# UofgCoastline/EUSIPCO-2026-Robust-Unet

Hardware: AMD Instinct MI355X
Metric: train images/sec Robust U-Net 256x256 bs16/GPU (higher is better)
Workload: dtype f32; 1 GPU; Robust U-Net base64 (40.9M params) train step, 256x256 RGB+mask tiles, batch 16/GPU, fp32, BCE + Adam(lr 1e-4, wd 1e-4), dropout + batch-stat BN on; global_batch=16, image_size=256, parallelism=dp1

## Files before the change

### eusipco-2026-robust-unet_amd/ops.py

```python
from __future__ import annotations

import ctypes
import os
import threading
import weakref

import torch

from ._lib import check, lib

CONV_FWD, CONV_DGRAD, CONVT_FWD, CONVT_DGRAD, CONV_DGRAD_T, CONVT_DGRAD_T = 0, 1, 2, 3, 4, 5

_ws = {}
PIN_SCRATCH = False
_retired = []


def grow(pool, key, nfloats, device, floor):
    buf = pool.get(key)
    if buf is None or buf.numel() < nfloats:
        if buf is not None and PIN_SCRATCH:
            _retired.append(buf)
        buf = torch.empty(max(int(nfloats), floor, 2 * buf.numel() if buf is not None else 0), device=device, dtype=torch.float32)
        if getattr(_tls, "override", None) is not None:
# ... 298 lines not shown
        return False
    return (USE_WINOGRAD4 and kh == 3 and cin_w == k and max(k, n) >= WINO4_MIN_WIDE and min(k, n) >= WINO4_MIN_NARROW and h * w <= WINO4_MAX_PIXELS
            and bool(lib.runet_wino4_supported(h // dil, w // dil, k, n)))


USE_STEM_KERNELS = os.environ.get("RUNET_NO_STEM_KERNELS", "0") != "1"


def _stem_case(cin, cin_w, cout, kh, dil=1):
    return USE_STEM_KERNELS and cin == 4 and kh in (1, 3) and dil == 1 and bool(lib.runet_stem_supported(cin_w, cout))


def stem_conv(x, w3, w1=None, stats3=None, stats1=None):
    n, h, w, _ = x.shape
    _, _, cin_w, cout = w3.shape
    y3 = empty_nhwc(n, h, w, cout, x)
    y1 = empty_nhwc(n, h, w, cout, x) if w1 is not None else None
    args = (x.data_ptr(), ld(x), w3.data_ptr(), w1.data_ptr() if w1 is not None else None, y3.data_ptr(), ld(y3),
            y1.data_ptr() if y1 is not None else None, ld(y1) if y1 is not None else 0, n, h, w, cin_w, cout)
    if EPILOGUE_STATS and stats3 is not None and (w1 is None or stats1 is not None):
        parts = lib.runet_stem_conv_stats_parts(n, h, w)
        s3 = _stats_buf(stats3, parts, cout, x.device)
        s1 = _stats_buf(stats1, parts, cout, x.device) if w1 is not None else None
        check(lib.runet_stem_conv_stats(*args, s3, s1, stream()))
    else:
        check(lib.runet_stem_conv(*args, stream()))
    return y3, y1


USE_CONV_X3 = os.environ.get("RUNET_NO_CONV_X3", "0") != "1"
CONV_X3_MIN_K = int(os.environ.get("RUNET_CONV_X3_MIN_K", "128"))
CONV_X3_WIDE_N = int(os.environ.get("RUNET_CONV_X3_WIDE_N", "128"))
CONVT_X3_NARROW = os.environ.get("RUNET_NO_CONVT_X3_NARROW", "0") != "1"
_X3_KIND = {CONV_FWD: "cx3f", CONV_DGRAD: "cx3d", CONVT_FWD: "cx3uf", CONVT_DGRAD: "cx3ud"}


def _conv_x3_case(x, cin, cin_w, cout, taps=1):
    k = cin * taps
    return (USE_X3 and USE_CONV_X3 and _PRECISION == "f32" and cin_w == cin and cin % 16 == 0 and cout % 4 == 0 and k >= CONV_X3_MIN_K
            and (k >= 2 * CONV_X3_MIN_K or cout >= CONV_X3_WIDE_N) and ld(x) % 4 == 0 and x.data_ptr() % 16 == 0)


def conv_x3_weights(w_hwio, mode):
    _, _, ci, co = w_hwio.shape
    k, n = (co, ci) if mode in (CONV_DGRAD, CONVT_DGRAD) else (ci, co)
    wp, dev = w_hwio.data_ptr(), w_hwio.device

    def make(out):
        buf = out if out is not None else torch.empty(lib.runet_conv_x3_pack_elems(k, n, mode), device=dev, dtype=torch.bfloat16)
        check(lib.runet_conv_x3_pack(wp, buf.data_ptr(), k, n, mode, stream()))
        return buf
    return _cached(w_hwio, _X3_KIND[mode], make, desc=(DERIVE_PACK, wp, k, n, mode))


EPILOGUE_STATS = os.environ.get("RUNET_NO_EPILOGUE_STATS", "0") != "1"


def _stats_buf(stats, nparts, c, dev):
    part = torch.empty(nparts * c * 3, device=dev, dtype=torch.float32)
    stats["part"], stats["nparts"] = part, nparts
    return part.data_ptr()


def _conv_x3(mode, x, w_hwio, bias, out, n, h, w, cin, cout, accumulate, stats=None):
    wp = conv_x3_weights(w_hwio, mode)
    prof = _PROFILE is not None
    if prof:
        e0, e1 = torch.cuda.Event(enable_timing=True), torch.cuda.Event(enable_timing=True)
        e0.record()
    if stats is not None and EPILOGUE_STATS and mode == CONV_FWD:
        sp = _stats_buf(stats, lib.runet_conv_x3_stats_parts(n, h, w), cout, x.device)
        check(lib.runet_conv_x3_stats(x.data_ptr(), ld(x), wp.data_ptr(), bias.data_ptr() if bias is not None else None, out.data_ptr(), ld(out), n, h, w,
                                      cin, cout, mode, int(accumulate), sp, stream()))
    else:
        check(lib.runet_conv_x3(x.data_ptr(), ld(x), wp.data_ptr(), bias.data_ptr() if bias is not None else None, out.data_ptr(), ld(out), n, h, w,
                                cin, cout, mode, int(accumulate), stream()))
    if prof:
        e1.record()
        fl = 2.0 * n * h * w * (4 if mode in (CONVT_FWD, CONVT_DGRAD) else 1) * cin * cout
        _PROFILE.append((lib.runet_conv_x3_kernel_name(n, h, w, cout, mode).decode(), fl, fl, e0, e1))
    return out


def conv_fwd(x, w_hwio, bias=None, out=None, dil=1, accumulate=False, keep_v=None, stats=None, pre=None):
    n, h, w, cin = x.shape
    kh, kw, cin_w, cout = w_hwio.shape
    if pre is not None:
        assert fuses_act_input(x, w_hwio) and dil == 1
        return wino4_conv(x, wino4_weights(w_hwio), bias, out=out, accumulate=accumulate, keep_v=keep_v, dil=dil, pre=pre, stats=stats)
    if _bf16_case(cin, cin_w):
        if out is None:
            out = empty_nhwc(n, h, w, cout, x)
        return _igemm_bf16(CONV_FWD, x, w_hwio, bias, out, n, h, w, cin, cout, kh, kw, dil, accumulate, False)
    if _wino4_case(h, w, kh, dil, cin, cout, cin_w):
        return wino4_conv(x, wino4_weights(w_hwio), bias, out=out, accumulate=accumulate, keep_v=keep_v, dil=dil, stats=stats)
    if _wino_case(h, w, kh, dil, cin, cout, cin_w, n, ld(x), ld(out) if out is not None else cout):
        return wino_conv(x, wino_weights(w_hwio), bias, out=out, accumulate=accumulate, stats=stats)
    if out is None:
        out = empty_nhwc(n, h, w, cout, x)
    if kh == 1 and _conv_x3_case(x, cin, cin_w, cout):
        return _conv_x3(CONV_FWD, x, w_hwio, bias, out, n, h, w, cin, cout, accumulate, stats=stats)
    _igemm(CONV_FWD, x.data_ptr(), ld(x), w_hwio.data_ptr(), bias.data_ptr() if bias is not None else None,
           out.data_ptr(), ld(out), n, h, w, cin, cin_w, cout, kh, kw, dil, int(accumulate))
    return out


USE_WINO_X3 = os.environ.get("RUNET_NO_WINO_X3", "0") != "1"


def wino_weights(w_hwio, dgrad=False):
    _, _, cin, cout = w_hwio.shape
    k, n = (cout, cin) if dgrad else (cin, cout)
    wp, dev = w_hwio.data_ptr(), w_hwio.device
    if USE_X3 and USE_WINO_X3 and k % 16 == 0:
        def make_x3(out):
            Up = out if out is not None else torch.empty(lib.runet_wino_x3_pack_elems(k, n), device=dev, dtype=torch.bfloat16)
            check(lib.runet_wino_weights_x3(wp, Up.data_ptr(), cin, cout, int(dgrad), stream()))
            Up.kn = (k, n)
            return Up
        return _cached(w_hwio, "wino2xd" if dgrad else "wino2x", make_x3, desc=(DERIVE_WINO2, wp, cin, cout, int(dgrad)))

    def make(out):
        U = out if out is not None else torch.empty((16, k, n), device=dev, dtype=torch.float32)
        check(lib.runet_wino_weights(wp, U.data_ptr(), cin, cout, int(dgrad), stream()))
        return U
    return _cached(w_hwio, "wino2d" if dgrad else "wino2", make)


def wino_conv(x, U, bias=None, out=None, accumulate=False, stats=None):
    n, h, w, k = x.shape
    x3 = U.dtype == torch.bfloat16
    nn_ = U.kn[1] if x3 else U.shape[2]
    if out is None:
        out = empty_nhwc(n, h, w, nn_, x)
    if _PROFILE is not None:
        e0, e1 = torch.cuda.Event(enable_timing=True), torch.cuda.Event(enable_timing=True)
        e0.record()
    if x3 and stats is not None and EPILOGUE_STATS:
        sp = _stats_buf(stats, lib.runet_wino_conv_x3_stats_parts(n, h, w), nn_, x.device)
        check(lib.runet_wino_conv_x3_stats(x.data_ptr(), ld(x), U.data_ptr(), bias.data_ptr() if bias is not None else None, out.data_ptr(), ld(out),
                                           n, h, w, k, nn_, int(accumulate), sp, stream()))
    else:
        fn = lib.runet_wino_conv_x3 if x3 else lib.runet_wino_conv
        check(fn(x.data_ptr(), ld(x), U.data_ptr(), bias.data_ptr() if bias is not None else None, out.data_ptr(), ld(out),
                 n, h, w, k, nn_, int(accumulate), stream()))
    if _PROFILE is not None:
        e1.record()
        fl = 2.0 * n * h * w * 9 * k * nn_
        _PROFILE.append(("wino_conv_x3_kernel" if x3 else "wino_conv_kernel", fl, fl * 16.0 / 36.0, e0, e1))
    return out


def wino_ok(h, w, cin, cout):
    return bool(lib.runet_wino_supported(h, w, cin, cout))


FUSE_BN_INPUT = os.environ.get("RUNET_NO_FUSED_BN_INPUT", "0") != "1"


def fuses_act_input(t, w_hwio):
    n, h, w, cin = t.shape
    kh, kw, cin_w, cout = w_hwio.shape
    return FUSE_BN_INPUT and not _bf16_case(cin, cin_w) and _wino4_case(h, w, kh, 1, cin, cout, cin_w)


def fuses_bn_bwd_input(dy, w_hwio):
    n, h, w, cout = dy.shape
    kh, kw, cin, cout_w = w_hwio.shape
    return (FUSE_BN_INPUT and cout_w == cout and not _bf16_case(cout, cout) and _wino4_case(h, w, kh, 1, cout, cin, cout) and USE_W4_ADJOINT
            and _x3_case(cout) and cin >= 16)


def conv_dgrad(dy, w_hwio, out=None, dil=1, accumulate=False, keep_z=None, bn=None):
    n, h, w, cout = dy.shape
    kh, kw, cin, cout_w = w_hwio.shape
    assert cout_w == cout
    if bn is not None:
        assert fuses_bn_bwd_input(dy, w_hwio) and dil == 1 and keep_z is not None
        return wino4_dgrad_adj(dy, w_hwio, out=out, accumulate=accumulate, dil=dil, keep_z=keep_z, bn=bn)
    if _bf16_case(cout, cout):
        if out is None:
            out = empty_nhwc(n, h, w, cin, dy)
        return _igemm_bf16(CONV_DGRAD, dy, w_hwio, None, out, n, h, w, cout, cin, kh, kw, dil, accumulate, True)
    if _wino4_case(h, w, kh, dil, cout, cin, cout):
        if USE_W4_ADJOINT and _x3_case(cout):
            return wino4_dgrad_adj(dy, w_hwio, out=out, accumulate=accumulate, dil=dil, keep_z=keep_z)
        return wino4_conv(dy, wino4_weights(w_hwio, dgrad=True), None, out=out, accumulate=accumulate, dil=dil)
    if _wino_case(h, w, kh, dil, cout, cin, cout, n, ld(dy), ld(out) if out is not None else cin):
        return wino_conv(dy, wino_weights(w_hwio, dgrad=True), None, out=out, accumulate=accumulate)
    if out is None:
        out = empty_nhwc(n, h, w, cin, dy)
    if kh == 1 and _conv_x3_case(dy, cout, cout, cin):
        return _conv_x3(CONV_DGRAD, dy, w_hwio, None, out, n, h, w, cout, cin, accumulate)
    if USE_TRANSPOSED_DGRAD:
        _igemm(CONV_DGRAD_T, dy.data_ptr(), ld(dy), transposed_weights(w_hwio).data_ptr(), None, out.data_ptr(), ld(out), n, h, w,
               cout, cout, cin, kh, kw, dil, int(accumulate))
    else:
        _igemm(CONV_DGRAD, dy.data_ptr(), ld(dy), w_hwio.data_ptr(), None, out.data_ptr(), ld(out), n, h, w,
               cout, cout, cin, kh, kw, dil, int(accumulate))
    return out


USE_WGRAD_STREAM = os.environ.get("RUNET_NO_WGRAD_STREAM", "0") != "1"
GRAPH_SIDE = os.environ.get("RUNET_GRAPH_SIDE", "0") == "1"
SIDE_RECORD_STREAM = os.environ.get("RUNET_SIDE_RECORD_STREAM", "0") == "1"
_side = {}


class wgrad_side_stream:

    def __enter__(self):
        if USE_WGRAD_STREAM and torch.cuda.is_available() and (GRAPH_SIDE or not torch.cuda.is_current_stream_capturing()):
            dev = torch.cuda.current_device()
            if ("s", dev) not in _side:
                _side[("s", dev)] = torch.cuda.Stream(device=dev)
            _side["active"] = _side[("s", dev)]
            _side["active_raw"] = _side["active"].cuda_stream
            _side["torch_switch"] = torch.cuda.is_current_stream_capturing()
        return self

    def __exit__(self, *exc):
        s = _side.pop("active", None)
        if s is not None:
            torch.cuda.current_stream().wait_stream(s)
        _side.pop("keep", None)
        return False


def side_stream():
    return _side.get("active")


FWD_BRANCHES = os.environ.get("RUNET_FWD_BRANCHES", "1") != "0"
BRANCH_MIN_PIXELS = int(os.environ.get("RUNET_BRANCH_MIN_PIXELS", str(1 << 18)))
_branch_now = True


def branches_pay(n, h, w):
    global _branch_now
    _branch_now = n * h * w >= BRANCH_MIN_PIXELS
    return _branch_now


class side_branch:

    def __init__(self, enabled=True):
        self.s = None
        if (enabled and FWD_BRANCHES and _branch_now and USE_WGRAD_STREAM and torch.cuda.is_available() and _side.get("active") is None
                and not torch.cuda.is_current_stream_capturing()):
            dev = torch.cuda.current_device()
            if ("s", dev) not in _side:
                _side[("s", dev)] = torch.cuda.Stream(device=dev)
            self.s = _side[("s", dev)]

    def __enter__(self):
        if self.s is not None:
            self.s.wait_stream(torch.cuda.current_stream())
            self.ctx = torch.cuda.stream(self.s)
            self.ctx.__enter__()
        return self

    def __exit__(self, *exc):
        if self.s is not None:
            self.ctx.__exit__(*exc)
        return False

    def join(self, *tensors):
        if self.s is not None:
            cur = torch.cuda.current_stream()
            cur.wait_stream(self.s)
            for t in tensors:
                if t is not None and (SIDE_RECORD_STREAM or getattr(t, "_runet_main_pool", False) is False):
                    t.record_stream(cur)
            self.s = None


def main_pool(t):
    t._runet_main_pool = True
    return t


def _on_side(fn, tensors):
    s = _side.get("active")
    if s is None:
        return fn()
    if _PROFILE is not None or _side.get("torch_switch"):
        s.wait_stream(torch.cuda.current_stream())
        with torch.cuda.stream(s):
            r = fn()
    else:
        raw = _side["active_raw"]
        check(lib.runet_stream_wait(raw, stream()))
        _tls.override = raw
        try:
            r = fn()
        finally:
            _tls.override = None
    if SIDE_RECORD_STREAM:
        for t in tensors:
            if t is not None:
                t.record_stream(s)
        return r
    keep = _side.setdefault("keep", [])
    for t in tensors:
        if t is not None:
            keep.append(t)
    return r


def conv_wgrad(x, dy, kh, kw, cin_w=None, dil=1, out=None, v=None, on_side=True, z=None):
    if on_side and _side.get("active") is not None:
        if out is None:
            out = torch.empty((kh, kw, x.shape[3] if cin_w is None else cin_w, dy.shape[3]), device=x.device, dtype=torch.float32)
        return _on_side(lambda: _conv_wgrad(x, dy, kh, kw, cin_w, dil, out, v, z), (x, dy, out, v, z))
    return _conv_wgrad(x, dy, kh, kw, cin_w, dil, out, v, z)


def _conv_wgrad(x, dy, kh, kw, cin_w=None, dil=1, out=None, v=None, z=None):
    n, h, w, cin = x.shape
    cout = dy.shape[3]
    cin_w = cin if cin_w is None else cin_w
    if out is None:
        out = torch.empty((kh, kw, cin_w, cout), device=x.device, dtype=torch.float32)
    if _bf16_case(cin, cin_w):
        return _wgrad_bf16(x, dy, out, n, h, w, cin, cout, kh, kw, dil, 0)
    if _wino4_case(h, w, kh, dil, cin, cout, cin_w) and cout >= 16:
        return wino4_wgrad(x, dy, out=out, v=v, dil=dil, z=z)
    if _stem_case(cin, cin_w, cout, kh, dil):
        ws = workspace(lib.runet_stem_wgrad_workspace_floats(n, h, w, cin_w, cout, kh), x.device)
        check(lib.runet_stem_wgrad(x.data_ptr(), ld(x), dy.data_ptr(), ld(dy), out.data_ptr(), ws.data_ptr(), ws.numel(), n, h, w, cin_w, cout, kh,
                                   stream()))
        return out
    prof = _PROFILE is not None
    if prof:
        e0, e1 = torch.cuda.Event(enable_timing=True), torch.cuda.Event(enable_timing=True)
        e0.record()
    if USE_WINOGRAD and kh == 3 and dil == 1 and cin_w == cin and h % 2 == 0 and w % 2 == 0 and cin >= 16:
        name = "wino_wgrad_direct_kernel(+reduce)"
        nws = lib.runet_wino_wgrad_workspace_floats(n, h, w, cin, cout)
        ws = workspace(nws, x.device)
        check(lib.runet_wino_wgrad(x.data_ptr(), ld(x), dy.data_ptr(), ld(dy), out.data_ptr(), ws.data_ptr(), ws.numel(), n, h, w, cin, cout, stream()))
    else:
        name = "wgrad_tile_kernel/wgrad_kernel(+reduce)"
        nws = lib.runet_conv_wgrad_workspace_floats(n, h, w, cin_w, cout, kh, kw)
        ws = workspace(nws, x.device)
        check(lib.runet_conv_wgrad(x.data_ptr(), ld(x), dy.data_ptr(), ld(dy), out.data_ptr(), ws.data_ptr(), ws.numel(),
                                   n, h, w, cin, cin_w, cout, kh, kw, dil, 0, stream()))
    if prof:
        e1.record()
        fl = 2.0 * n * h * w * kh * kw * cin_w * cout
        _PROFILE.append((name, fl, fl * 16.0 / 36.0 if name.startswith("wino") else fl, e0, e1))
    return out


def _wgrad_bf16(x, dy, out, n, h, w, cin, cout, kh, kw, dil, transposed):
    prof = _PROFILE is not None
    if prof:
        e0, e1 = torch.cuda.Event(enable_timing=True), torch.cuda.Event(enable_timing=True)
        e0.record()
    nws = _lp("runet_conv_wgrad_{}_workspace_floats")(n, h, w, cin, cout, kh, kw, dil, transposed)
    ws = workspace(nws, x.device)
    check(_lp("runet_conv_wgrad_{}")(x.data_ptr(), ld(x), dy.data_ptr(), ld(dy), out.data_ptr(), ws.data_ptr(), ws.numel(), n, h, w, cin, cout,
                                    kh, kw, dil, transposed, stream()))
    if prof:
        e1.record()
        fl = 2.0 * n * h * w * kh * kw * cin * cout
        nbytes = 4.0 * n * h * w * (cin + (4 if transposed else 1) * cout) + 4.0 * kh * kw * cin * cout
        _PROFILE.append((f"wgrad_{_PRECISION}_kernel", fl, fl, e0, e1, nbytes))
    return out


def convt_fwd(x, w_hwio, bias=None, out=None):
    n, h, w, cin = x.shape
    _, _, cin_w, cout = w_hwio.shape
    if out is None:
        out = empty_nhwc(n, 2 * h, 2 * w, cout, x)
    if _bf16_case(cin, cin_w):
        return _igemm_bf16(CONVT_FWD, x, w_hwio, bias, out, n, h, w, cin, cout, 2, 2, 1, False, False)
    if _conv_x3_case(x, cin, cin_w, cout) or (CONVT_X3_NARROW and cout >= 32 and _conv_x3_case(x, cin, cin_w, max(cout, CONV_X3_WIDE_N))):
        return _conv_x3(CONVT_FWD, x, w_hwio, bias, out, n, h, w, cin, cout, False)
    _igemm(CONVT_FWD, x.data_ptr(), ld(x), w_hwio.data_ptr(), bias.data_ptr() if bias is not None else None,
           out.data_ptr(), ld(out), n, h, w, cin, cin_w, cout, 2, 2, 1, 0)
    return out


def convt_dgrad(dy, w_hwio, out=None, accumulate=False):
    n, h2, w2, cout = dy.shape
    _, _, cin, cout_w = w_hwio.shape
    h, w = h2 // 2, w2 // 2
    if out is None:
        out = empty_nhwc(n, h, w, cin, dy)
    if _bf16_case(cout, cout):
        return _igemm_bf16(CONVT_DGRAD, dy, w_hwio, None, out, n, h, w, cout, cin, 2, 2, 1, accumulate, True)
    if _conv_x3_case(dy, cout, cout, cin, taps=4):
        return _conv_x3(CONVT_DGRAD, dy, w_hwio, None, out, n, h, w, cout, cin, accumulate)
    if USE_TRANSPOSED_DGRAD:
        _igemm(CONVT_DGRAD_T, dy.data_ptr(), ld(dy), transposed_weights(w_hwio).data_ptr(), None, out.data_ptr(), ld(out), n, h, w,
               cout, cout, cin, 2, 2, 1, int(accumulate))
    else:
        _igemm(CONVT_DGRAD, dy.data_ptr(), ld(dy), w_hwio.data_ptr(), None, out.data_ptr(), ld(out), n, h, w,
               cout, cout, cin, 2, 2, 1, int(accumulate))
    return out


def convt_wgrad(x, dy, out=None):
    if _side.get("active") is not None:
        if out is None:
            out = torch.empty((2, 2, x.shape[3], dy.shape[3]), device=x.device, dtype=torch.float32)
        return _on_side(lambda: _convt_wgrad(x, dy, out), (x, dy, out))
    return _convt_wgrad(x, dy, out)


def _convt_wgrad(x, dy, out=None):
    n, h, w, cin = x.shape
    cout = dy.shape[3]
    if out is None:
        out = torch.empty((2, 2, cin, cout), device=x.device, dtype=torch.float32)
    if _bf16_case(cin, cin):
        return _wgrad_bf16(x, dy, out, n, h, w, cin, cout, 2, 2, 1, 1)
    nws = lib.runet_conv_wgrad_workspace_floats(n, h, w, cin, cout, 2, 2)
    ws = workspace(nws, x.device)
    check(lib.runet_conv_wgrad(x.data_ptr(), ld(x), dy.data_ptr(), ld(dy), out.data_ptr(), ws.data_ptr(), ws.numel(),
                               n, h, w, cin, cin, cout, 2, 2, 1, 1, stream()))
    return out
# ... 467 lines not shown
```

### include/runet_hip.h

```cpp
#ifndef RUNET_HIP_H
#define RUNET_HIP_H
#ifdef __cplusplus
extern "C" {
#endif

const char* runet_last_error(void);
void runet_set_error(const char* msg);
int runet_abi_version(void);

enum { RUNET_CONV_FWD = 0, RUNET_CONV_DGRAD = 1, RUNET_CONVT_FWD = 2, RUNET_CONVT_DGRAD = 3, RUNET_CONV_DGRAD_T = 4, RUNET_CONVT_DGRAD_T = 5 };

int runet_conv_igemm(const float* x, int ldx, const float* w, const float* bias, float* y, int ldy,
                     int n_img, int h, int w_, int cin, int cin_w, int cout, int kh, int kw, int dil,
                     int mode, int accumulate, void* stream);

int runet_transpose_taps(const float* w, float* wt, int taps, int cin, int cout, void* stream);

const char* runet_conv_igemm_kernel_name(int n_img, int h, int w_, int cin, int cout, int kh, int mode);
int runet_igemm_force_variant(int variant);
int runet_igemm_lowp_force_variant(int variant);

long runet_conv_wgrad_workspace_floats(int n_img, int h, int w_, int cin_w, int cout, int kh, int kw);
int runet_conv_wgrad(const float* x, int ldx, const float* dy, int ldy, float* dw, float* workspace,
                     long workspace_floats, int n_img, int h, int w_, int cin, int cin_w, int cout,
// ... 65 lines not shown
int runet_sa_conv7_bwd(const float* smap, const float* dq, const float* wp, float* dsm, float* dwp, float* workspace, int n_img, int h,
                       int w, void* stream);
int runet_rb_bwd2(const float* dv, int lddv, const float* t2, int ld, const float* sa, const float* dsm, const int* amax, int n_img,
                  int hw, int c, float* workspace, float* sdu, float* sdut, void* stream);
long runet_rb_bwd2_bn_workspace_floats(int n_img, int hw, int c);
int runet_rb_bwd2_bn(const float* dv, int lddv, const float* t2, int ld, const float* sa, const float* dsm, const int* amax, const float* r, int ldr,
                     const float* mean_s, const float* invstd_s, int n_img, int hw, int c, float* workspace, long workspace_floats, float* sdu,
                     float* sdut, float* sums_s, void* stream);
long runet_ca_bwd_workspace_floats(int n_img, int c, int cr);
int runet_ca_bwd(const float* sdu, const float* sdut, const float* s2, const float* h2, const float* ca, const float* avg, const float* mx,
                 const float* w0p, const float* w2p, const float* mean_nc, const float* tval, const float* mean2, const float* invstd2,
                 int n_img, int c, int cr, float* workspace, float* davg, float* dmx, float* sums2, float* dw0p, float* dw2p, void* stream);
int runet_rb_bwd3(const float* dv, int lddv, const float* t2, int ld, const float* sa, const float* dsm, const int* amax, const float* ca,
                  const float* davg, const float* dmx, const int* idx, const float* mean2, const float* invstd2, const float* s2,
                  const float* sums2, float* dt2, int lddt, long pixels, int hw, int c, long m_total, void* stream);
int runet_rb_bwd3_sc(float* dv, int lddv, const float* t2, int ld, const float* sa, const float* dsm, const int* amax, const float* ca,
                     const float* davg, const float* dmx, const int* idx, const float* mean2, const float* invstd2, const float* s2,
                     const float* sums2, float* dt2, int lddt, const float* r, int ldr, const float* mean_s, const float* invstd_s,
                     const float* scale_s, const float* sums_s, long m_total_s, long pixels, int hw, int c, long m_total, void* stream);

int runet_ag_psi(const float* g1, int ldg, const float* x1, int ldx, const float* sg, const float* hg, const float* sx, const float* hx,
                 const float* wpsi, const float* bpsi, float* s, long pixels, int f, void* stream);
int runet_ag_out(const float* xs, int ldx, const float* s, const float* sp, const float* hp, float* out, int ldo, long pixels, int c,
                 void* stream);
int runet_ag_bwd1(const float* datt, int ldd, const float* xs, int ldx, const float* s, const float* sp, const float* hp, float* dxs,
                  int lddx, float* dsbn, long pixels, int c, void* stream);
int runet_ag_bwd2(const float* ds, const float* g1, int ldg, const float* x1, int ldx, const float* sg, const float* hg, const float* sx,
                  const float* hx, const float* wpsi, float* dpre, int ldp, float* workspace, float* dwpsi_db, long pixels, int f,
                  void* stream);
long runet_ag_bwd2_bn_workspace_floats(long pixels, int f);
int runet_ag_bwd2_bn(const float* ds, const float* g1, int ldg, const float* x1, int ldx, const float* sg, const float* hg, const float* sx,
                     const float* hx, const float* wpsi, const float* mean_g, const float* invstd_g, const float* mean_x, const float* invstd_x,
                     float* dpre, int ldp, float* workspace, long workspace_floats, float* dwpsi_db, float* sums_g, float* sums_x, long pixels, int f,
                     void* stream);

int runet_outc_fwd(const float* x, int ld, const float* w, const float* b, float* logit, float* prob, long pixels, int c, void* stream);
int runet_outc_bwd(const float* dprob, const float* prob, const float* x, int ld, const float* w, float* dx, int lddx, float* workspace,
                   float* dw_db, long pixels, int c, void* stream);

int runet_maxpool2_fwd(const float* x, int ldx, float* y, int ldy, unsigned char* idx, int n_img, int h, int w, int c, void* stream);
int runet_maxpool2_bwd(const float* dy, int lddy, const unsigned char* idx, float* dx, int lddx, int n_img, int h, int w, int c,
                       int accumulate, void* stream);
int runet_to_nhwc_pad(const float* x, long sn, long sc, long sh, long sw, float* y, int n_img, int c, int h, int w, int c_pad, void* stream);

int runet_bce_fwd(const float* prob, const float* target, long n, double* workspace1024, float* loss, void* stream);
int runet_bce_bwd(const float* prob, const float* target, const float* grad_out, float* dprob, long n, void* stream);

int runet_adam_chunk_elems(void);
int runet_adam_multi(const long long* table, int n_tensors, const int* chunks, int n_chunks, float lr, float beta1, float beta2, float eps,
                     float weight_decay, int step, float grad_scale, const int* skip_flag, void* stream);

int runet_adam_multi_dev(const long long* table, int n_tensors, const int* chunks, int n_chunks, const float* hyper, int* step_dev,
                         const int* skip_flag, void* stream);
int runet_nonfinite_flag(const float* buf, long n, int* flag2, void* stream);
int runet_stream_wait(void* waiter, void* waited);


int runet_seg_counts(const float* pred, const float* target, long long* counts, int n_img, long per_img, float threshold, void* stream);

int runet_gemm_batched(const float* a, int lda, long stride_a, const float* b, long stride_b, float* c, int ldc, long stride_c, int batch, int rows,
                       int k, int n, void* stream);
int runet_gemm_tn_batched(const float* a, int lda, long stride_a, const float* b, int ldb, long stride_b, float* c, int batch, int rows, int k, int n,
                          int rows_per_split, void* stream);
const char* runet_gemm_batched_kernel_name(int batch, int rows, int k, int n);

int runet_gemm_x3_supported(int rows, int k, int n);
long runet_gemm_x3_pack_elems(int batch, int k, int n);
int runet_gemm_x3_pack(const float* b, long stride_b, void* packed, int batch, int k, int n, void* stream);
int runet_gemm_x3_batched(const float* a, int lda, long stride_a, const void* packed_b, float* c, int ldc, long stride_c, int batch, int rows,
                          int k, int n, void* stream);
int runet_gemm_x3_tn_batched(const float* a, int lda, long stride_a, const float* b, int ldb, long stride_b, float* c, int batch, int rows, int k,
                             int n, int rows_per_split, void* stream);
const char* runet_gemm_x3_kernel_name(int batch, int rows, int k, int n);
int runet_gemm_x3_tn_convt(const float* x, int ldx, const float* dy, int ldy, float* c, int n_img, int h, int w, int cin, int cout,
                           int rows_per_split, void* stream);

int runet_conv_x3_supported(int cin, int cout, int mode);
long runet_conv_x3_pack_elems(int cin, int cout, int mode);
int runet_conv_x3_pack(const float* w, void* packed, int cin, int cout, int mode, void* stream);
int runet_conv_x3(const float* x, int ldx, const void* wpacked, const float* bias, float* y, int ldy, int n_img, int h, int w, int cin, int cout,
                  int mode, int accumulate, void* stream);
const char* runet_conv_x3_kernel_name(int n_img, int h, int w, int cout, int mode);

enum { RUNET_DERIVE_WINO4 = 0, RUNET_DERIVE_WINO2 = 1, RUNET_DERIVE_PACK = 2 };
int runet_derive_desc_bytes(void);
int runet_derive_desc(void* host_table, int index, int kind, const float* w, void* dst, int cin, int cout, int mode, int first_block);
int runet_derive_multi(const void* table, int n_desc, int total_blocks, void* stream);
int runet_conv_x3_stats_parts(int n_img, int h, int w);
int runet_conv_x3_stats(const float* x, int ldx, const void* wpacked, const float* bias, float* y, int ldy, int n_img, int h, int w, int cin, int cout,
                        int mode, int accumulate, float* stats, void* stream);

int runet_wino4_supported(int h, int w, int k, int n);
long runet_wino4_workspace_floats(int n_img, int h, int w, int k, int n);
int runet_wino4_weights(const float* w_hwio, float* U, int cin, int cout, int dgrad, void* stream);
int runet_wino4_conv(const float* x, int ldx, const float* U, const float* bias, float* y, int ldy, int n_img, int h, int w, int k, int n,
                     int dil, int accumulate, float* workspace, long workspace_floats, void* stream);
int runet_wino4_weights_x3(const float* w_hwio, void* Upacked, int cin, int cout, int dgrad, void* stream);
int runet_wino4_conv_x3(const float* x, int ldx, const void* Upacked, const float* bias, float* y, int ldy, int n_img, int h, int w, int k, int n,
                        int dil, int accumulate, float* workspace, long workspace_floats, void* stream);
int runet_wino4_input(const float* src, int ld, int c, int n_img, int h, int w, int dil, int mode, float* V, void* stream);
int runet_wino4_input_act(const float* t, int ld, int c, int n_img, int h, int w, int dil, const float* scale, const float* shift,
                          const float* factor_nc, float* V, void* stream);
int runet_wino4_input_bn_bwd(const float* dy, int lddy, const float* x, int ldx, int c, int n_img, int h, int w, int dil, const float* mean,
                             const float* invstd, const float* scale, const float* shift, const float* sums, const float* factor_nc,
                             long m_total, float* Z, void* stream);
int runet_wino4_output(const float* M, int n, int n_img, int h, int w, int dil, const float* bias, float* y, int ldy, int accumulate, void* stream);
int runet_wino4_output_stats_parts(int n_img, int h, int w, int n, int dil);
int runet_wino4_output_stats(const float* M, int n, int n_img, int h, int w, const float* bias, float* y, int ldy, int accumulate, float* stats, void* stream);
int runet_wino4_output_adj(const float* M, int n, int n_img, int h, int w, int dil, float* y, int ldy, int accumulate, void* stream);
int runet_wino4_wgrad_output(const float* dU, int splits, int cin, int cout, float* dw, void* stream);
int runet_wino4_wgrad_rows_per_split(int n_img, int h, int w, int cin, int cout);
long runet_wino4_wgrad_workspace_floats(int n_img, int h, int w, int cin, int cout);
int runet_wino4_wgrad(const float* x, int ldx, const float* dy, int ldy, float* dw, float* workspace, long workspace_floats, int n_img, int h, int w,
                      int cin, int cout, int dil, void* stream);

int runet_stem_supported(int cin_w, int cout);
int runet_stem_conv(const float* x, int ldx, const float* w3, const float* w1, float* y3, int ldy3, float* y1, int ldy1, int n_img,
                    int h, int w, int cin_w, int cout, void* stream);
int runet_stem_conv_stats_parts(int n_img, int h, int w);
int runet_stem_conv_stats(const float* x, int ldx, const float* w3, const float* w1, float* y3, int ldy3, float* y1, int ldy1, int n_img,
                          int h, int w, int cin_w, int cout, float* stats3, float* stats1, void* stream);
long runet_stem_wgrad_workspace_floats(int n_img, int h, int w, int cin_w, int cout, int ksize);
int runet_stem_wgrad(const float* x, int ldx, const float* dy, int ldy, float* dw, float* workspace, long workspace_floats, int n_img,
                     int h, int w, int cin_w, int cout, int ksize, void* stream);

int runet_conv2d_general(const float* x, int ldx, const float* w, const float* bias, float* y, int ldy, int n_img, int hin, int win, int cin,
                         int cin_w, int cout, int kh, int kw, int stride, int pad, int dil, int mode, int accumulate, void* stream);
int runet_convt4_igemm(const float* x, int ldx, const float* w, const float* bias, float* y, int ldy, int n_img, int h, int w_, int cin, int cout,
                       int mode, int accumulate, void* stream);
long runet_conv_wgrad_general_workspace_floats(int pixels, int cin_w, int cout, int kh, int kw);
int runet_conv_wgrad_general(const float* x, int ldx, const float* dy, int ldy, float* dw, float* workspace, long workspace_floats, int n_img,
                             int hin, int win, int cin, int cin_w, int cout, int kh, int kw, int stride, int pad, int dil, int transposed4,
                             void* stream);
int runet_maxpool3s2_fwd(const float* x, int ldx, float* y, int ldy, unsigned char* idx, int n_img, int h, int w, int c, void* stream);
int runet_maxpool3s2_bwd(const float* dy, int lddy, const unsigned char* idx, float* dx, int lddx, int n_img, int h, int w, int c, void* stream);
int runet_add_inplace(float* dst, const float* src, long n, void* stream);
int runet_broadcast_nc(const float* v_nc, float* y, int ldy, int n_img, int hw, int c, void* stream);
int runet_head3x3_fwd(const float* x, int ld, const float* w, const float* b, float* prob, int n_img, int h, int w_, int c, void* stream);
long runet_head3x3_bwd_workspace_floats(int n_img, int h, int w_, int c);
int runet_head3x3_bwd(const float* dprob, const float* prob, const float* x, int ld, const float* w, float* dx, int lddx, float* workspace,
                      float* dw_db, int n_img, int h, int w_, int c, void* stream);


long runet_bf16_pack_elems(int taps, int k, int n);
int runet_bf16_pack_weights(const float* w_hwio, void* packed, int taps, int cin, int cout, int transpose, void* stream);
int runet_conv_igemm_bf16(const float* x, int ldx, const void* wpacked, const float* bias, float* y, int ldy, int n_img, int h, int w_,
                          int cin, int cout, int kh, int kw, int dil, int mode, int accumulate, void* stream);
long runet_conv_wgrad_bf16_workspace_floats(int n_img, int h, int w_, int cin, int cout, int kh, int kw, int dil, int transposed);
int runet_conv_wgrad_bf16(const float* x, int ldx, const float* dy, int ldy, float* dw, float* workspace, long workspace_floats,
                          int n_img, int h, int w_, int cin, int cout, int kh, int kw, int dil, int transposed, void* stream);

long runet_fp16_pack_elems(int taps, int k, int n);
int runet_fp16_pack_weights(const float* w_hwio, void* packed, int taps, int cin, int cout, int transpose, void* stream);
int runet_conv_igemm_fp16(const float* x, int ldx, const void* wpacked, const float* bias, float* y, int ldy, int n_img, int h, int w_,
                          int cin, int cout, int kh, int kw, int dil, int mode, int accumulate, void* stream);
long runet_conv_wgrad_fp16_workspace_floats(int n_img, int h, int w_, int cin, int cout, int kh, int kw, int dil, int transposed);
int runet_conv_wgrad_fp16(const float* x, int ldx, const float* dy, int ldy, float* dw, float* workspace, long workspace_floats,
                          int n_img, int h, int w_, int cin, int cout, int kh, int kw, int dil, int transposed, void* stream);

int runet_bilinear_fwd(const float* x, float* y, long planes, int h, int w, int ho, int wo, void* stream);
int runet_bilinear_bwd(const float* dy, float* dx, long planes, int h, int w, int ho, int wo, void* stream);
int runet_mul_pixel(const float* x, int ldx, const float* s, float* y, int ldy, long pixels, int c, void* stream);

int runet_nhwc_to_nchw(const float* x, int ld, float* y, int n_img, int c, long hw, void* stream);
int runet_ce_fwd(const float* logits_nchw, const long long* target, int n_img, int classes, long hw, double* partials1024, float* loss, void* stream);
int runet_ce_bwd(const float* logits_nchw, const long long* target, const float* gout, float* dlogits_nchw, int n_img, int classes, long hw,
// ... 175 lines not shown
```

Measured before the change: 598.7 images/s.

## Add persistent streaming MFMA kernels for 1x1 conv forward, dgrad and wgrad

Adds a persistent kernel for f32 1x1 convolutions (forward and dgrad). Each block keeps the whole weight matrix in LDS, and each wave streams 32-pixel tiles through MFMA with the next tile's activations prefetched into registers. This replaces the generic implicit-GEMM path for small channel counts that the x3 path does not cover. A separate wgrad kernel, which reduces per-block slabs and then sums them in double, is added but only runs when an environment flag is set.

```diff
diff --git a/eusipco-2026-robust-unet_amd/csrc/conv1x1_stream.hip b/eusipco-2026-robust-unet_amd/csrc/conv1x1_stream.hip
--- /dev/null
+++ b/eusipco-2026-robust-unet_amd/csrc/conv1x1_stream.hip
@@ -0,0 +1,460 @@
+#include "runet_common.h"
+#include <stdlib.h>
+#include "../../include/runet_hip.h"
+
+namespace {
+
+struct StreamArgs {
+    const float* x; int ldx;
+    const float* w; int w_sk, w_sn;
+    const float* bias;
+    float* y; int ldy;
+    long P;
+    long ntiles;
+    int cout, accumulate;
+};
+
+template <int KC, int TN>
+constexpr int stream_min_blocks() { return (16 * KC + 32 * TN <= 200) ? 2 : 1; }
+
+template <int KC, int TN, bool ACC>
+__global__ __launch_bounds__(256, (stream_min_blocks<KC, TN>())) void conv1x1_stream_kernel(StreamArgs g) {
+    constexpr int NC = 2 * KC;
+    extern __shared__ __attribute__((aligned(16))) float wl[];
+
+    const int tid = threadIdx.x, lane = tid & 63;
+    const int wid = __builtin_amdgcn_readfirstlane(tid >> 6);
+    const int li = lane & 31, lh = lane >> 5;
+    const int cin = 16 * KC;
+
+    float bv[TN];
+#pragma unroll
+    for (int b = 0; b < TN; ++b) bv[b] = (g.bias != nullptr && b * 32 + li < g.cout) ? g.bias[b * 32 + li] : 0.f;
+    const bool last_ok = (TN - 1) * 32 + li < g.cout;
+
+    const long nwaves = (long)gridDim.x * 4;
+    const long t_last = g.ntiles - 1;
+    const unsigned ldy4 = (unsigned)g.ldy * 4u;
+    const unsigned y_lane4 = (unsigned)(4 * lh) * ldy4 + (unsigned)li * 4u;
+
+    auto rows_of = [&](long t) -> int {
+        const long left = g.P - t * 32;
+        return left < 32 ? (int)left : 32;
+    };
+    auto y_rsrc = [&](long t) {
+        const int rows = rows_of(t);
+        return __builtin_amdgcn_make_buffer_rsrc(g.y + t * 32 * g.ldy, 0, (int)(((unsigned)(rows - 1) * (unsigned)g.ldy + (unsigned)g.cout) * 4u), 0x00020000);
+    };
+    auto load_a = [&](f32x4 (&a)[NC], long t) {
+        const int rows = rows_of(t);
+        const int row = li < rows ? li : rows - 1;
+        const float* ab = g.x + t * 32 * g.ldx;
+        const unsigned off = (unsigned)row * (unsigned)g.ldx + (unsigned)(4 * lh);
+#pragma unroll
+        for (int c = 0; c < NC; ++c) a[c] = ld4(ab + (off + 8u * c));
+    };
+    auto load_old = [&](float (&old)[TN][16], long t) {
+        const __amdgpu_buffer_rsrc_t ry = y_rsrc(t);
+        int yl = (int)y_lane4;
+        asm volatile("" : "+v"(yl));
+#pragma unroll
+        for (int r = 0; r < 16; ++r) {
+            const int vo = yl + ((r & 3) + 8 * (r >> 2)) * (int)ldy4;
+#pragma unroll
+            for (int b = 0; b < TN; ++b) old[b][r] = __builtin_bit_cast(float, __builtin_amdgcn_raw_buffer_load_b32(ry, vo + 128 * b, 0, 0));
+        }
+    };
+
+    float old[TN][16];
+#pragma unroll
+    for (int b = 0; b < TN; ++b)
+#pragma unroll
+        for (int r = 0; r < 16; ++r) old[b][r] = 0.f;
+
+    auto step = [&](f32x4 (&a_cur)[NC], f32x4 (&a_nxt)[NC], long t) {
+        const long tn = t + nwaves < t_last ? t + nwaves : t_last;
+        load_a(a_nxt, tn);
+        __builtin_amdgcn_sched_barrier(0);
+        f32x16 acc[TN];
+#pragma unroll
+        for (int b = 0; b < TN; ++b)
+#pragma unroll
+            for (int r = 0; r < 16; ++r) acc[b][r] = 0.f;
+        int wl_lane = lane;
+        asm volatile("" : "+v"(wl_lane));
+        const int wlane = wl_lane * 4;
+#pragma unroll
+        for (int c = 0; c < NC; ++c) {
+            f32x4 bf[TN];
+#pragma unroll
+            for (int b = 0; b < TN; ++b) bf[b] = *reinterpret_cast<const f32x4*>(wl + (c * TN + b) * 256 + wlane);
+#pragma unroll
+            for (int q = 0; q < 4; ++q)
+#pragma unroll
+                for (int b = 0; b < TN; ++b) acc[b] = __builtin_amdgcn_mfma_f32_32x32x2f32(a_cur[c][q], bf[b][q], acc[b], 0, 0, 0);
+        }
+        __builtin_amdgcn_sched_barrier(0);
+        const __amdgpu_buffer_rsrc_t ry = y_rsrc(t);
+        int yl = (int)y_lane4;
+        asm volatile("" : "+v"(yl));
+#pragma unroll
+        for (int r = 0; r < 16; ++r) {
+            const int vo = yl + ((r & 3) + 8 * (r >> 2)) * (int)ldy4;
+#pragma unroll
+            for (int b = 0; b < TN - 1; ++b)
+                __builtin_amdgcn_raw_buffer_store_b32(__builtin_bit_cast(unsigned, acc[b][r] + bv[b] + old[b][r]), ry, vo + 128 * b, 0, 0);
+        }
+        if (last_ok) {
+            constexpr int b = TN - 1;
+#pragma unroll
+            for (int r = 0; r < 16; ++r) {
+                const int vo = yl + ((r & 3) + 8 * (r >> 2)) * (int)ldy4;
+                __builtin_amdgcn_raw_buffer_store_b32(__builtin_bit_cast(unsigned, acc[b][r] + bv[b] + old[b][r]), ry, vo + 128 * b, 0, 0);
+            }
+        }
+        __builtin_amdgcn_sched_barrier(0);
+        if constexpr (ACC) load_old(old, tn);
+    };
+
+    long t = (long)blockIdx.x * 4 + wid;
+    f32x4 a0[NC], a1[NC];
+    {
+        const long t0 = t < t_last ? t : t_last;
+        load_a(a0, t0);
+        if constexpr (ACC) load_old(old, t0);
+    }
+    if (g.cout < 32 * TN) {
+        for (int e = tid; e < NC * TN * 256; e += 256) wl[e] = 0.f;
+        lds_barrier();
+    }
+    {
+        constexpr int MAXV = (KC * TN + 1) / 2;
+        const int total4 = cin * g.cout / 4;
+        const bool ncontig = g.w_sn == 1;
+        const int cq = g.cout >> 2;
+        auto widx = [&](int k, int n) { return (((k >> 3) * TN + (n >> 5)) * 64 + ((k >> 2) & 1) * 32 + (n & 31)) * 4 + (k & 3); };
+#pragma unroll
+        for (int i0 = 0; i0 < MAXV; i0 += 4) {
+            f32x4 v[4];
+#pragma unroll
+            for (int j = 0; j < 4; ++j) {
+                const int e4 = tid + 256 * (i0 + j);
+                if (i0 + j < MAXV && e4 < total4) v[j] = ld4(g.w + 4 * (long)e4);
+            }
+#pragma unroll
+            for (int j = 0; j < 4; ++j) {
+                const int e4 = tid + 256 * (i0 + j);
+                if (i0 + j < MAXV && e4 < total4) {
+                    if (ncontig) {
+                        const int k = e4 / cq, n = (e4 - k * cq) * 4;
+#pragma unroll
+                        for (int q = 0; q < 4; ++q) wl[widx(k, n + q)] = v[j][q];
+                    } else {
+                        const int n = e4 / (cin / 4), k = (e4 - n * (cin / 4)) * 4;
+                        st4(wl + widx(k, n), v[j]);
+                    }
+                }
+            }
+        }
+    }
+    lds_barrier();
+    if (t >= g.ntiles) return;
+    for (;;) {
+        step(a0, a1, t);
+        t += nwaves;
+        if (t >= g.ntiles) break;
+        step(a1, a0, t);
+        t += nwaves;
+        if (t >= g.ntiles) break;
+    }
+}
+
+template <int KC, int TN>
+void launch_stream(const StreamArgs& a, int blocks, hipStream_t st) {
+    const size_t lds = (size_t)2 * KC * TN * 256 * sizeof(float);
+    if (a.accumulate) hipLaunchKernelGGL((conv1x1_stream_kernel<KC, TN, true>), dim3(blocks), dim3(256), lds, st, a);
+    else hipLaunchKernelGGL((conv1x1_stream_kernel<KC, TN, false>), dim3(blocks), dim3(256), lds, st, a);
+}
+
+template <int KC>
+void dispatch_tn(const StreamArgs& a, int blocks, hipStream_t st) {
+    switch ((a.cout + 31) / 32) {
+    case 1: launch_stream<KC, 1>(a, blocks, st); break;
+    case 2: launch_stream<KC, 2>(a, blocks, st); break;
+    case 3: launch_stream<KC, 3>(a, blocks, st); break;
+    default: launch_stream<KC, 4>(a, blocks, st); break;
+    }
+}
+
+int stream_cu_count() {
+    static const int cus = [] {
+        int dev = 0, n = 0;
+        if (hipGetDevice(&dev) != hipSuccess || hipDeviceGetAttribute(&n, hipDeviceAttributeMultiprocessorCount, dev) != hipSuccess || n <= 0) n = 256;
+        return n;
+    }();
+    return cus;
+}
+
+bool stream_shape_ok(int cin, int cout, int mode) {
+    return (mode == RUNET_CONV_FWD || mode == RUNET_CONV_DGRAD) && cin >= 16 && cin <= 128 && cin % 16 == 0 && cout >= 4 && cout <= 128 && cout % 4 == 0;
+}
+
+}
+
+extern "C" int runet_conv1x1_stream_supported(int cin, int cout, int mode) { return stream_shape_ok(cin, cout, mode) ? 1 : 0; }
+
+extern "C" int runet_conv1x1_stream_blocks(int n_img, int h, int w_, int cin, int cout) {
+    if (n_img <= 0 || h <= 0 || w_ <= 0 || cin <= 0 || cout <= 0) return 0;
+    const char* e = getenv("RUNET_CONV1X1_STREAM_BLOCKS");
+    const int forced = e ? atoi(e) : 0;
+    if (forced > 0) return forced < 65535 ? forced : 65535;
+    const int per_cu = (cin + (cout + 31) / 32 * 32 <= 200) ? 2 : 1;
+    const long tiles = ((long)n_img * h * w_ + 31) / 32;
+    long blocks = (long)stream_cu_count() * per_cu;
+    const long need = (tiles + 3) / 4;
+    if (blocks > need) blocks = need;
+    return (int)(blocks < 1 ? 1 : blocks);
+}
+
+extern "C" const char* runet_conv1x1_stream_kernel_name(int cin, int cout, int accumulate) {
+    static thread_local char name[64];
+    snprintf(name, sizeof(name), "conv1x1_stream_kernel<%d, %d, %s>", cin / 16, (cout + 31) / 32, accumulate ? "true" : "false");
+    return name;
+}
+
+extern "C" int runet_conv1x1_stream(const float* x, int ldx, const float* w, const float* bias, float* y, int ldy, int n_img, int h, int w_,
+                                    int cin, int cout, int mode, int accumulate, void* stream) {
+    RUNET_REQUIRE(x && w && y, "null pointer");
+    RUNET_REQUIRE(stream_shape_ok(cin, cout, mode), "needs mode FWD or DGRAD, cin a multiple of 16 and cout a multiple of 4, both <= 128");
+    RUNET_REQUIRE(ldx >= cin && ldx % 4 == 0 && ldy >= cout && ldy % 4 == 0, "pixel strides must be multiples of 4 floats and cover the channels");
+    RUNET_REQUIRE(((uintptr_t)x % 16) == 0 && ((uintptr_t)w % 16) == 0 && ((uintptr_t)y % 16) == 0, "pointers must be 16-byte aligned");
+    RUNET_REQUIRE(n_img > 0 && h > 0 && w_ > 0, "empty iteration space");
+    StreamArgs a{};
+    a.x = x; a.ldx = ldx; a.w = w; a.bias = bias; a.y = y; a.ldy = ldy;
+    a.P = (long)n_img * h * w_;
+    a.ntiles = (a.P + 31) / 32;
+    a.cout = cout; a.accumulate = accumulate != 0;
+    if (mode == RUNET_CONV_FWD) { a.w_sk = cout; a.w_sn = 1; }
+    else { a.w_sk = 1; a.w_sn = cin; }
+    const int blocks = runet_conv1x1_stream_blocks(n_img, h, w_, cin, cout);
+    hipStream_t st = (hipStream_t)stream;
+    switch (cin / 16) {
+    case 1: dispatch_tn<1>(a, blocks, st); break;
+    case 2: dispatch_tn<2>(a, blocks, st); break;
+    case 3: dispatch_tn<3>(a, blocks, st); break;
+    case 4: dispatch_tn<4>(a, blocks, st); break;
+    case 5: dispatch_tn<5>(a, blocks, st); break;
+    case 6: dispatch_tn<6>(a, blocks, st); break;
+    case 7: dispatch_tn<7>(a, blocks, st); break;
+    default: dispatch_tn<8>(a, blocks, st); break;
+    }
+    RUNET_CHECK_LAUNCH();
+}
+
+
+namespace {
+
+struct WgStreamArgs {
+    const float* x; int ldx;
+    const float* dy; int ldy;
+    float* slabs;
+    long P, chunk;
+    int cin, cout;
+};
+
+template <int V>
+__device__ __forceinline__ void wg_load(float (&v)[V], const float* base, int ld, int q, int np) {
+    typedef float f32x2 __attribute__((ext_vector_type(2)));
+    const int qc = q < np ? q : (np > 0 ? np - 1 : 0);
+    const float* p = base + (long)qc * ld;
+    if constexpr (V == 1) {
+        v[0] = *p;
+    } else if constexpr (V == 2) {
+        const f32x2 t = *reinterpret_cast<const f32x2*>(p);
+        v[0] = t[0]; v[1] = t[1];
+    } else {
+        const f32x4 t = ld4(p);
+#pragma unroll
+        for (int e = 0; e < 4; ++e) v[e] = t[e];
+    }
+}
+
+template <int VA, int VB, bool TR>
+__global__ __launch_bounds__(256, 2) void conv1x1_wgrad_stream_kernel(WgStreamArgs g) {
+    constexpr int S = VA * VB >= 8 ? 4 : 8;
+    extern __shared__ __attribute__((aligned(16))) float red[];
+    const int tid = threadIdx.x, lane = tid & 63;
+    const int wid = __builtin_amdgcn_readfirstlane(tid >> 6);
+    const int li = lane & 31, lh = lane >> 5;
+
+    const long p0 = ((long)blockIdx.x * 4 + wid) * g.chunk;
+    long np = g.P - p0;
+    np = np < g.chunk ? np : g.chunk;
+    np = np > 0 ? np : 0;
+    const long pb = np > 0 ? p0 : 0;
+    const int npi = (int)np;
+    const float* xl = g.x + pb * g.ldx + VA * li;
+    const float* yl = g.dy + pb * g.ldy + VB * li;
+    const int nb = (int)((np + 2 * S - 1) / (2 * S));
+
+    f32x16 acc[VA][VB];
+#pragma unroll
+    for (int a = 0; a < VA; ++a)
+#pragma unroll
+        for (int b = 0; b < VB; ++b)
+#pragma unroll
+            for (int r = 0; r < 16; ++r) acc[a][b][r] = 0.f;
+
+    auto load_batch = [&](float (&A)[S][VA], float (&B)[S][VB], int bi) {
+#pragma unroll
+        for (int s = 0; s < S; ++s) {
+            wg_load<VA>(A[s], xl, g.ldx, bi * 2 * S + 2 * s + lh, npi);
+            wg_load<VB>(B[s], yl, g.ldy, bi * 2 * S + 2 * s + lh, npi);
+        }
+    };
+    auto mma_batch = [&](float (&A)[S][VA], float (&B)[S][VB], int bi) {
+#pragma unroll
+        for (int s = 0; s < S; ++s) {
+            const bool ok = bi * 2 * S + 2 * s + lh < npi;
+#pragma unroll
+            for (int a = 0; a < VA; ++a) {
+                const float av = ok ? A[s][a] : 0.f;
+#pragma unroll
+                for (int b = 0; b < VB; ++b) acc[a][b] = __builtin_amdgcn_mfma_f32_32x32x2f32(av, ok ? B[s][b] : 0.f, acc[a][b], 0, 0, 0);
+            }
+        }
+    };
+
+    float A0[S][VA], B0[S][VB], A1[S][VA], B1[S][VB];
+    load_batch(A0, B0, 0);
+    for (int bi = 0; bi < nb; bi += 2) {
+        load_batch(A1, B1, bi + 1);
+        __builtin_amdgcn_sched_barrier(0);
+        mma_batch(A0, B0, bi);
+        __builtin_amdgcn_sched_barrier(0);
+        load_batch(A0, B0, bi + 2);
+        __builtin_amdgcn_sched_barrier(0);
+        mma_batch(A1, B1, bi + 1);
+        __builtin_amdgcn_sched_barrier(0);
+    }
+
+    constexpr int CA = 32 * VA, CB = 32 * VB, n_out = CA * CB;
+    float* rl = red + (VA * 4 * lh) * CB + VB * li;
+    auto to_lds = [&](bool first) {
+#pragma unroll
+        for (int a = 0; a < VA; ++a)
+#pragma unroll
+            for (int b = 0; b < VB; ++b)
+#pragma unroll
+                for (int r = 0; r < 16; ++r) {
+                    float* o = rl + (VA * ((r & 3) + 8 * (r >> 2)) + a) * CB + b;
+                    *o = first ? acc[a][b][r] : *o + acc[a][b][r];
+                }
+    };
+    if (wid == 0) to_lds(true);
+    lds_barrier();
+#pragma unroll 1
+    for (int wv = 1; wv < 4; ++wv) {
+        if (wid == wv) to_lds(false);
+        lds_barrier();
+    }
+    float* slab = g.slabs + (long)blockIdx.x * n_out;
+    if constexpr (!TR) {
+        for (int e = tid * 4; e < n_out; e += 1024) st4(slab + e, ld4(red + e));
+    } else {
+        for (int e = tid; e < n_out; e += 256) slab[e] = red[(e % CA) * CB + e / CA];
+    }
+}
+
+__global__ __launch_bounds__(256) void wgrad_slab_sum_kernel(const float* __restrict__ slabs, int nslabs, int n, float* __restrict__ out) {
+    __shared__ double part[256][4];
+    const int col = threadIdx.x & 31, kl = threadIdx.x >> 5;
+    const long i = ((long)blockIdx.x * 32 + col) * 4;
+    double s[4] = {0., 0., 0., 0.};
+    if (i < n)
+        for (int k = kl; k < nslabs; k += 8) {
+            const f32x4 v = ld4(slabs + (long)k * n + i);
+#pragma unroll
+            for (int e = 0; e < 4; ++e) s[e] += v[e];
+        }
+#pragma unroll
+    for (int e = 0; e < 4; ++e) part[threadIdx.x][e] = s[e];
+    __syncthreads();
+    if (kl == 0 && i < n) {
+#pragma unroll
+        for (int j = 1; j < 8; ++j)
+#pragma unroll
+            for (int e = 0; e < 4; ++e) s[e] += part[j * 32 + col][e];
+        const f32x4 r = {(float)s[0], (float)s[1], (float)s[2], (float)s[3]};
+        st4(out + i, r);
+    }
+}
+
+bool wgrad_stream_shape_ok(int cin, int cout) {
+    auto w = [](int c) { return c == 32 || c == 64 || c == 128; };
+    return w(cin) && w(cout) && (cin < 128 || cout < 128);
+}
+
+void wgrad_stream_plan(long P, int& slabs, long& chunk) {
+    long b = (P + 255) / 256;
+    b = b < 1 ? 1 : (b > 256 ? 256 : b);
+    slabs = (int)b;
+    chunk = ((P + b * 4 - 1) / (b * 4) + 15) / 16 * 16;
+}
+
+template <int VA, int VB, bool TR>
+void wg_launch(const WgStreamArgs& a, int blocks, hipStream_t st) {
+    hipLaunchKernelGGL((conv1x1_wgrad_stream_kernel<VA, VB, TR>), dim3(blocks), dim3(256), (size_t)a.cin * a.cout * sizeof(float), st, a);
+}
+
+template <bool TR>
+void wg_dispatch(const WgStreamArgs& a, int blocks, hipStream_t st) {
+    const int va = a.cin / 32, vb = a.cout / 32;
+    if (va == 1) wg_launch<1, 1, TR>(a, blocks, st);
+    else if (va == 2 && vb == 1) wg_launch<2, 1, TR>(a, blocks, st);
+    else if (va == 2) wg_launch<2, 2, TR>(a, blocks, st);
+    else if (vb == 1) wg_launch<4, 1, TR>(a, blocks, st);
+    else wg_launch<4, 2, TR>(a, blocks, st);
+}
+
+}
+
+extern "C" int runet_conv1x1_wgrad_stream_supported(int cin, int cout) { return wgrad_stream_shape_ok(cin, cout) ? 1 : 0; }
+
+extern "C" int runet_conv1x1_wgrad_stream_slabs(int n_img, int h, int w_) {
+    if (n_img <= 0 || h <= 0 || w_ <= 0) return 0;
+    int slabs; long chunk;
+    wgrad_stream_plan((long)n_img * h * w_, slabs, chunk);
+    return slabs;
+}
+
+extern "C" long runet_conv1x1_wgrad_stream_workspace_floats(int n_img, int h, int w_, int cin, int cout) {
+    if (cin <= 0 || cout <= 0) return 0;
+    return (long)runet_conv1x1_wgrad_stream_slabs(n_img, h, w_) * cin * cout;
+}
+
+extern "C" int runet_conv1x1_wgrad_stream(const float* x, int ldx, const float* dy, int ldy, float* dw, float* workspace, long workspace_floats,
+                                          int n_img, int h, int w_, int cin, int cout, void* stream) {
+    RUNET_REQUIRE(x && dy && dw && workspace, "null pointer");
+    RUNET_REQUIRE(wgrad_stream_shape_ok(cin, cout), "needs cin and cout of 32, 64 or 128, not both 128");
+    RUNET_REQUIRE(ldx >= cin && ldx % 4 == 0 && ldy >= cout && ldy % 4 == 0, "pixel strides must be multiples of 4 floats and cover the channels");
+    RUNET_REQUIRE(((uintptr_t)x % 16) == 0 && ((uintptr_t)dy % 16) == 0 && ((uintptr_t)dw % 16) == 0 && ((uintptr_t)workspace % 16) == 0,
+                  "pointers must be 16-byte aligned");
+    RUNET_REQUIRE(n_img > 0 && h > 0 && w_ > 0, "empty iteration space");
+    WgStreamArgs a{};
+    a.x = x; a.ldx = ldx; a.dy = dy; a.ldy = ldy; a.slabs = workspace; a.cin = cin; a.cout = cout;
+    a.P = (long)n_img * h * w_;
+    int slabs;
+    wgrad_stream_plan(a.P, slabs, a.chunk);
+    RUNET_REQUIRE(workspace_floats >= (long)slabs * cin * cout, "workspace too small (runet_conv1x1_wgrad_stream_workspace_floats)");
+    RUNET_REQUIRE(a.chunk < (1L << 30), "a wave's pixel range exceeds 32-bit pixel indices");
+    hipStream_t st = (hipStream_t)stream;
+    if (cout > cin) {
+        a.x = dy; a.ldx = ldy; a.dy = x; a.ldy = ldx; a.cin = cout; a.cout = cin;
+        wg_dispatch<true>(a, slabs, st);
+    } else {
+        wg_dispatch<false>(a, slabs, st);
+    }
+    hipLaunchKernelGGL(wgrad_slab_sum_kernel, dim3(cdiv(cin * cout, 128)), dim3(256), 0, st, workspace, slabs, cin * cout, dw);
+    RUNET_CHECK_LAUNCH();
+}
diff --git a/eusipco-2026-robust-unet_amd/ops.py b/eusipco-2026-robust-unet_amd/ops.py
--- a/eusipco-2026-robust-unet_amd/ops.py
+++ b/eusipco-2026-robust-unet_amd/ops.py
@@ -404,6 +404,30 @@
     return out
 
 
+USE_CONV1X1_STREAM = os.environ.get("RUNET_NO_CONV1X1_STREAM", "0") != "1"
+
+
+def _conv1x1_stream_case(mode, x, cin, cin_w, cout, kh=1, kw=1, out=None):
+    return (USE_CONV1X1_STREAM and _PRECISION == "f32" and kh == 1 and kw == 1 and cin_w == cin
+            and bool(lib.runet_conv1x1_stream_supported(cin, cout, mode)) and not _conv_x3_case(x, cin, cin_w, cout)
+            and ld(x) % 4 == 0 and x.data_ptr() % 16 == 0 and (out is None or (ld(out) % 4 == 0 and out.data_ptr() % 16 == 0)))
+
+
+def _conv1x1_stream(mode, x, w_hwio, bias, out, n, h, w, cin, cout, accumulate):
+    args = (x.data_ptr(), ld(x), w_hwio.data_ptr(), bias.data_ptr() if bias is not None else None, out.data_ptr(), ld(out), n, h, w, cin, cout,
+            mode, int(accumulate), stream())
+    if _PROFILE is None:
+        check(lib.runet_conv1x1_stream(*args))
+        return out
+    e0, e1 = torch.cuda.Event(enable_timing=True), torch.cuda.Event(enable_timing=True)
+    e0.record()
+    check(lib.runet_conv1x1_stream(*args))
+    e1.record()
+    fl = 2.0 * n * h * w * cin * cout
+    _PROFILE.append((lib.runet_conv1x1_stream_kernel_name(cin, cout, int(accumulate)).decode(), fl, fl, e0, e1))
+    return out
+
+
 def conv_fwd(x, w_hwio, bias=None, out=None, dil=1, accumulate=False, keep_v=None, stats=None, pre=None):
     n, h, w, cin = x.shape
     kh, kw, cin_w, cout = w_hwio.shape
@@ -422,6 +446,8 @@
         out = empty_nhwc(n, h, w, cout, x)
     if kh == 1 and _conv_x3_case(x, cin, cin_w, cout):
         return _conv_x3(CONV_FWD, x, w_hwio, bias, out, n, h, w, cin, cout, accumulate, stats=stats)
+    if dil == 1 and _conv1x1_stream_case(CONV_FWD, x, cin, cin_w, cout, kh, kw, out):
+        return _conv1x1_stream(CONV_FWD, x, w_hwio, bias, out, n, h, w, cin, cout, accumulate)
     _igemm(CONV_FWD, x.data_ptr(), ld(x), w_hwio.data_ptr(), bias.data_ptr() if bias is not None else None,
            out.data_ptr(), ld(out), n, h, w, cin, cin_w, cout, kh, kw, dil, int(accumulate))
     return out
@@ -514,6 +540,8 @@
         out = empty_nhwc(n, h, w, cin, dy)
     if kh == 1 and _conv_x3_case(dy, cout, cout, cin):
         return _conv_x3(CONV_DGRAD, dy, w_hwio, None, out, n, h, w, cout, cin, accumulate)
+    if dil == 1 and _conv1x1_stream_case(CONV_DGRAD, dy, cout, cout, cin, kh, kw, out):
+        return _conv1x1_stream(CONV_DGRAD, dy, w_hwio, None, out, n, h, w, cout, cin, accumulate)
     if USE_TRANSPOSED_DGRAD:
         _igemm(CONV_DGRAD_T, dy.data_ptr(), ld(dy), transposed_weights(w_hwio).data_ptr(), None, out.data_ptr(), ld(out), n, h, w,
                cout, cout, cin, kh, kw, dil, int(accumulate))
@@ -628,6 +656,16 @@
         if t is not None:
             keep.append(t)
     return r
+
+
+USE_CONV1X1_WGRAD_STREAM = (os.environ.get("RUNET_CONV1X1_WGRAD_STREAM", "0") == "1"
+                            and os.environ.get("RUNET_NO_CONV1X1_WGRAD_STREAM", "0") != "1")
+
+
+def _conv1x1_wgrad_stream_case(x, dy, cin, cin_w, cout, kh=1, kw=1, out=None):
+    return (USE_CONV1X1_WGRAD_STREAM and _PRECISION == "f32" and kh == 1 and kw == 1 and cin_w == cin
+            and bool(lib.runet_conv1x1_wgrad_stream_supported(cin, cout)) and ld(x) % 4 == 0 and x.data_ptr() % 16 == 0
+            and ld(dy) % 4 == 0 and dy.data_ptr() % 16 == 0 and (out is None or (out.is_contiguous() and out.data_ptr() % 16 == 0)))
 
 
 def conv_wgrad(x, dy, kh, kw, cin_w=None, dil=1, out=None, v=None, on_side=True, z=None):
@@ -662,6 +700,11 @@
         nws = lib.runet_wino_wgrad_workspace_floats(n, h, w, cin, cout)
         ws = workspace(nws, x.device)
         check(lib.runet_wino_wgrad(x.data_ptr(), ld(x), dy.data_ptr(), ld(dy), out.data_ptr(), ws.data_ptr(), ws.numel(), n, h, w, cin, cout, stream()))
+    elif dil == 1 and _conv1x1_wgrad_stream_case(x, dy, cin, cin_w, cout, kh, kw, out):
+        name = "conv1x1_wgrad_stream_kernel(+sum)"
+        ws = workspace(lib.runet_conv1x1_wgrad_stream_workspace_floats(n, h, w, cin, cout), x.device)
+        check(lib.runet_conv1x1_wgrad_stream(x.data_ptr(), ld(x), dy.data_ptr(), ld(dy), out.data_ptr(), ws.data_ptr(), ws.numel(), n, h, w, cin, cout,
+                                             stream()))
     else:
         name = "wgrad_tile_kernel/wgrad_kernel(+reduce)"
         nws = lib.runet_conv_wgrad_workspace_floats(n, h, w, cin_w, cout, kh, kw)
diff --git a/include/runet_hip.h b/include/runet_hip.h
--- a/include/runet_hip.h
+++ b/include/runet_hip.h
@@ -171,6 +171,17 @@
                   int mode, int accumulate, void* stream);
 const char* runet_conv_x3_kernel_name(int n_img, int h, int w, int cout, int mode);
 
+int runet_conv1x1_stream_supported(int cin, int cout, int mode);
+int runet_conv1x1_stream_blocks(int n_img, int h, int w, int cin, int cout);
+int runet_conv1x1_stream(const float* x, int ldx, const float* w, const float* bias, float* y, int ldy, int n_img, int h, int w_, int cin,
+                         int cout, int mode, int accumulate, void* stream);
+const char* runet_conv1x1_stream_kernel_name(int cin, int cout, int accumulate);
+int runet_conv1x1_wgrad_stream_supported(int cin, int cout);
+int runet_conv1x1_wgrad_stream_slabs(int n_img, int h, int w);
+long runet_conv1x1_wgrad_stream_workspace_floats(int n_img, int h, int w, int cin, int cout);
+int runet_conv1x1_wgrad_stream(const float* x, int ldx, const float* dy, int ldy, float* dw, float* workspace, long workspace_floats,
+                               int n_img, int h, int w_, int cin, int cout, void* stream);
+
 enum { RUNET_DERIVE_WINO4 = 0, RUNET_DERIVE_WINO2 = 1, RUNET_DERIVE_PACK = 2 };
 int runet_derive_desc_bytes(void);
 int runet_derive_desc(void* host_table, int index, int kind, const float* w, void* dst, int cin, int cout, int mode, int first_block);
```

Result: faster. 605.1 images/s, median of 6 (+1.1%).
